# EPFL-IMOS/simple-SFOD

Hardware: AMD Instinct MI355X
Metric: teacher+student train images/s on 1024x2048 synthetic (higher is better)
Workload: dtype bf16x3

## Files before the change

include/sfod_hip.h:

```cpp
#ifndef SFOD_HIP_H
#define SFOD_HIP_H
#include <stdint.h>
#ifdef __cplusplus
extern "C" {
#endif

#define SFOD_F32 0
#define SFOD_BF16 1
#define SFOD_BF16X3 2
#define SFOD_F16X3 3

int sfod_version(void);
const char* sfod_last_error(void);

int sfod_preprocess(const void* const* img_ptrs, const int32_t* sizes, int B, int Hp, int Wp,
                    int Cpad, const float* mean3, const float* std3, void* out, int dt,
                    void* stream);

int sfod_hflip_u8(const void* src, void* dst, int C, int H, int W, void* stream);

int sfod_resize_bilinear_u8(const void* src, void* dst, int C, int H, int W, int h, int w,
                            const int32_t* hbounds, const int32_t* hcoef, int ksize_h,
                            const int32_t* vbounds, const int32_t* vcoef, int ksize_v, int flip,
                            void* stream);
int sfod_resize_bilinear_u8_opt(const void* src, void* dst, int C, int H, int W, int y0, int x0, int ch, int cw,
                                int h, int w, const int32_t* hbounds, const int32_t* hcoef, int ksize_h,
                                const int32_t* vbounds, const int32_t* vcoef, int ksize_v, int flip_mode,
                                void* stream);

int sfod_mosaic_u8(const void* const* tiles, const void* const* tabs, const int32_t* geom, int n_tiles, int fill,
                   void* out, int H0, int W0, void* stream);

int sfod_conv_fwd(const void* x, const void* w, const float* bias, void* y, int B, int H, int W,
                  int Cin, int Cout, int ksize, int ldy, int act, float* stats, int dt, int out_dt,
                  void* stream);
int sfod_conv_fwd_ws(const void* x, const void* w, const uint32_t* w_absmax, const float* bias, void* y, int B, int H,
                     int W, int Cin, int Cout, int ksize, int ldy, int act, float* stats, int dt, int out_dt,
                     void* stream);
int64_t sfod_conv_fwd_scratch_bytes(int B, int H, int W, int Cin, int Cout, int ksize, int dt, int out_dt, int with_stats);
int sfod_conv_fwd_scratch(const void* x, const void* w, const uint32_t* w_absmax, const float* bias, void* y, int B, int H,
                          int W, int Cin, int Cout, int ksize, int ldy, int act, float* stats, int dt, int out_dt,
                          void* scratch, int64_t scratch_bytes, void* stream);
int sfod_conv_stats_blocks(int B, int H, int W, int Cin, int Cout, int ksize, int dt);
int sfod_set_conv_algo(int algo);
int sfod_conv_dgrad_bnred_blocks(int B, int H, int W, int Cin, int Cout, int dt);
int sfod_conv_dgrad_bnred(const void* x, const void* w, void* dz, int B, int H, int W, int Cin, int Cout, int dt,
                          const float* y, const float* mean, const float* invstd, const float* gamma,
                          const float* beta, float* red_ws, void* stream);
int sfod_conv_fwd_bnin_supported(int B, int H, int W, int Cin, int Cout, int dt);
int sfod_conv_fwd_bnin(const float* x_pre, const float* in_mean, const float* in_invstd, const float* in_gamma,
                       const float* in_beta, const void* w, const float* bias, float* y, int B, int H, int W, int Cin,
                       int Cout, int ldy, int act, float* stats, int dt, void* stream);
int sfod_set_gemm_tile(int tile);
int sfod_set_conv3x3_variant(int variant);
int sfod_last_conv_kernel(char* buf, int n);
int sfod_set_deterministic(int on);
int sfod_get_deterministic(void);
int sfod_set_conv3x3_m16(int on);
int sfod_set_wgrad3x3_pipe(int on);
int sfod_conv_fwd_algo(int B, int H, int W, int Cin, int Cout, int ksize, int dt);

int sfod_conv_first_supported(int B, int H, int W, int Cin, int Cout, int dt, int ldy);
int sfod_conv_first_fused(const void* x, const void* w, const float* bias, const float* scale,
                          const float* shift, void* y, float* stats, int B, int H, int W, int ldy,
                          int act, int dt, void* stream);
int sfod_conv_first_fused_ws(const void* x, const void* w, const uint32_t* w_absmax, const float* bias,
                             const float* scale, const float* shift, void* y, float* stats, int B, int H, int W,
                             int ldy, int act, int dt, void* stream);
int sfod_conv_first_stats_blocks(int B, int H, int W);
int sfod_set_conv_first_pipe(int on);
int sfod_set_conv_first_grid(int n);
int sfod_conv_first_bn_apply_supported(int B, int H, int W, int Cin, int Cout, int pool_flags, int dt, int y_dt);
int sfod_conv_first_bn_apply(const void* x, const void* w, const float* bias, const float* mean, const float* invstd,
                             const float* gamma, const float* beta, void* z, int B, int H, int W, int ldz, int dt,
                             void* stream);
int sfod_set_first_apply_recompute(int on);

int64_t sfod_conv_wgrad_ws_bytes(int B, int H, int W, int Cin, int Cout, int ksize, int lddy, int dt);
int sfod_conv_wgrad(const void* x, const void* dy, float* dw, int B, int H, int W, int Cin,
                    int Cout, int ksize, int lddy, int dt, void* ws, int64_t ws_bytes, void* stream);
int sfod_conv_wgrad_oihw_supported(int B, int H, int W, int Cin, int Cout, int ksize, int lddy, int dt);
int sfod_conv_wgrad_oihw(const void* x, const void* dy, float* dw_oihw, int B, int H, int W, int Cin,
                         int Cout, int ksize, int lddy, int dt, int accumulate, void* ws,
                         int64_t ws_bytes, void* stream);
int sfod_conv_first_wgrad_bn_supported(int B, int H, int W, int Cin, int Cout, int pool, int dt, int y_dt);
int sfod_conv_first_wgrad_bn(const void* x, const void* dz, const void* y, const float* mean, const float* invstd,
                             const float* gamma, const float* beta, const float* dgamma, const float* dbeta,
                             float* dw, int B, int H, int W, int Cin, int Cout, int dt, int oihw, int accumulate,
                             void* ws, int64_t ws_bytes, void* stream);
int sfod_set_first_wgrad_fused(int on);

int sfod_pack_conv_weight(const float* w_oihw, void* w_packed, int Cout, int Cin, int ksize,
                          int CinPad, int rot180, int dt, void* stream);
int sfod_pack_conv_weight_ws(const float* w_oihw, void* w_packed, uint32_t* absmax, int Cout, int Cin, int ksize,
                             int CinPad, int rot180, int dt, void* stream);
int sfod_pack_conv_weights_blocks(int Cout, int Cin, int ksize, int innerPad, int rot180);
int sfod_pack_conv_weights_multi(const int64_t* desc, int n, int total_blocks, int dt, void* stream);
int sfod_pack_conv_weights_multi_ws(const int64_t* desc, int n, int total_blocks, int dt, uint32_t* absmax ,
                                    void* stream);
int sfod_unpack_conv_wgrad(const float* dw_packed, float* dw_oihw, int Cout, int Cin, int ksize,
                           int CinPad, int accumulate, void* stream);
int sfod_pack_fc_weight(const float* w, void* out, int N, int K, int chw_c, int transpose, int dt,
                        void* stream);
int sfod_unpack_fc_wgrad(const float* dw_packed, float* dw, int N, int K, int chw_c,
                         int accumulate, void* stream);
int sfod_pack_fc_weight_ld(const float* w, void* out, int N, int K, int chw_c, int transpose, int ld,
                           int dt, void* stream);
int sfod_pack_fc_weight_ld_ws(const float* w, void* out, uint32_t* absmax, int N, int K, int chw_c, int transpose,
                              int ld, int dt, void* stream);
int sfod_unpack_fc_wgrad_ld(const float* dw_packed, float* dw, int N, int K, int chw_c, int ld,
                            int accumulate, void* stream);
int sfod_bias_grad(const void* dy, float* db, int M, int N, int ld, int accumulate, int dt,
                   void* stream);

int sfod_bn_finalize(const float* stats, int nblocks, int M, int C,
                     float* mean, float* invstd, float* running_mean, float* running_var,
                     float momentum, float eps, int update_running, int64_t* num_batches_tracked,
                     float* ws, void* stream);
int sfod_bn_finalize_pop(const float* stats, int nblocks, int M, int C,
                         float* mean, float* invstd, float* running_mean, float* running_var,
                         float momentum, float eps, int update_running, int64_t* num_batches_tracked,
                         float* ws, double* pop, int64_t pop_stride, void* stream);
int sfod_bn_pop_commit(const double* pop, int64_t pop_stride, const int64_t* table, const int64_t* table_host, int n,
                       void* stream);
int sfod_bn_pop_merge(double* dst, const double* src, int64_t columns, void* stream);
int sfod_set_bn_finalize_fused(int on);
int sfod_bn_finalize_ws_floats(int C);
int sfod_bn_relu_pool_fwd(const void* y, const float* mean, const float* invstd,
                          const float* gamma, const float* beta, void* z, int B, int H, int W,
                          int C, int pool, int dt, int out_dt, void* stream);
int sfod_bn_relu_pool_fwd2(const void* y, const float* mean, const float* invstd,
                           const float* gamma, const float* beta, void* z, void* z2, int B, int H, int W,
                           int C, int pool, int dt, int out_dt, void* stream);
int sfod_bn_add_relu_fwd(const void* y, const float* mean, const float* invstd, const float* gamma,
                         const float* beta, const void* residual, void* z, void* z_pairs, void* z_pairs2, int64_t rows,
                         int C, int dt, int pairs_dt, void* stream);
int sfod_bn_relu_pool_bwd(const void* dz, const void* y, const float* mean, const float* invstd,
                          const float* gamma, const float* beta, void* dy, float* dgamma,
                          float* dbeta, float* dgamma_acc, float* dbeta_acc, float* ws, int B, int H,
                          int W, int C, int pool, int dt, int out_dt, int reduced_blocks, void* stream);
#define SFOD_BN_BWD_SCRATCH_ROWS 32
// ... 233 lines not shown
```

simple-sfod_amd/csrc/conv3x3_patch.hip:

```cpp
#include "conv_internal.h"
#include <type_traits>
#include <stdlib.h>

typedef __attribute__((ext_vector_type(8))) __bf16 bf16x8;
typedef __attribute__((ext_vector_type(16))) float f32x16;
typedef __attribute__((ext_vector_type(4))) float f32x4_t;

#define LDS_PTR(p) ((__attribute__((address_space(3))) void*)(p))

namespace {

template <int J> using IC = std::integral_constant<int, J>;

constexpr int BSLOT = 8192;
constexpr int STG_PITCH = 144;

template <int G, int FM> struct Lay {
  static constexpr bool SMALL = (G == 1) ? (FM == 2) : (FM == 1);
  static constexpr int NPW = SMALL ? 3 : 5;
  static constexpr int PATCH_ROWS = NPW * 8 * 16;
  static constexpr int PATCH_BYTES = PATCH_ROWS * 64;
  static constexpr int D = SMALL ? 2 : 3;
  static constexpr int NBS = D + 1;
  static constexpr int BRING_OFF = 2 * PATCH_BYTES;
// ... 506 lines not shown
      }
    }
    if (lane == 0) scnt[wave] = (float)cnt;
    __syncthreads();
    if (threadIdx.x < BN) {
      const int col = threadIdx.x;
      const int cwn = (G == 1) ? (col >> 6) : 0;
      const int cl = col & 63;
      constexpr int NWM = (G == 1) ? 4 : 8;
      double n_tot = 0.0, s_tot = 0.0;
#pragma unroll
      for (int k = 0; k < NWM; ++k) {
        const int wv = (G == 1) ? (k * 2 + cwn) : k;
        n_tot += (double)scnt[wv];
        s_tot += (double)sred[(wv * 64 + cl) * 2 + 0];
      }
      const double mu = n_tot > 0.0 ? s_tot / n_tot : 0.0;
      double m2 = 0.0;
#pragma unroll
      for (int k = 0; k < NWM; ++k) {
        const int wv = (G == 1) ? (k * 2 + cwn) : k;
        const double nk = (double)scnt[wv];
        if (nk > 0.0) {
          const double d = (double)sred[(wv * 64 + cl) * 2 + 0] / nk - mu;
          m2 += (double)sred[(wv * 64 + cl) * 2 + 1] + nk * d * d;
        }
      }
      const int n = n0 + col;
      if (n < a.Cout) {
        a.stats[((int64_t)mtile * 2 + 0) * a.Cout + n] = (float)s_tot;
        a.stats[((int64_t)mtile * 2 + 1) * a.Cout + n] = (float)m2;
      }
      if (col == 0 && tn == 0) a.stats[(int64_t)a.nblk * 2 * a.Cout + mtile] = (float)n_tot;
    }
  }
}


template <int FMT>
__device__ __forceinline__ f32x4_t mfma16(bf16x8 a, bf16x8 b, f32x4_t c) {
  if constexpr (FMT == 2)
    return __builtin_amdgcn_mfma_f32_16x16x32_f16(__builtin_bit_cast(sfod_f16x8, a), __builtin_bit_cast(sfod_f16x8, b), c, 0, 0, 0);
  else
    return __builtin_amdgcn_mfma_f32_16x16x32_bf16(a, b, c, 0, 0, 0);
}

__device__ __forceinline__ float row16_sum(float v) {
  v += __builtin_bit_cast(float, __builtin_amdgcn_update_dpp(0, __builtin_bit_cast(int, v), 0xB1, 0xF, 0xF, true));
  v += __builtin_bit_cast(float, __builtin_amdgcn_update_dpp(0, __builtin_bit_cast(int, v), 0x4E, 0xF, 0xF, true));
  v += __builtin_bit_cast(float, __builtin_amdgcn_update_dpp(0, __builtin_bit_cast(int, v), 0x141, 0xF, 0xF, true));
  v += __builtin_bit_cast(float, __builtin_amdgcn_update_dpp(0, __builtin_bit_cast(int, v), 0x140, 0xF, 0xF, true));
  return v;
}

__device__ __forceinline__ void wait_vm_dyn(int n) {
  switch (n) {
    case 0: wait_vm<0>(); break;   case 1: wait_vm<1>(); break;   case 2: wait_vm<2>(); break;   case 3: wait_vm<3>(); break;
    case 4: wait_vm<4>(); break;   case 5: wait_vm<5>(); break;   case 6: wait_vm<6>(); break;   case 7: wait_vm<7>(); break;
    case 8: wait_vm<8>(); break;   case 9: wait_vm<9>(); break;   case 10: wait_vm<10>(); break; case 11: wait_vm<11>(); break;
    case 12: wait_vm<12>(); break; case 13: wait_vm<13>(); break; case 14: wait_vm<14>(); break; default: wait_vm<15>(); break;
  }
}

template <int NW, int NIP, int NWN = 2> struct M16Lay {
  static constexpr int PIX = (NW / NWN) * NIP * 16;
  static constexpr int PR = (PIX == 256) ? 384 : 640;
  static constexpr int NPW = PR / 16 / NW;
  static constexpr int PPS = (NPW + 2) / 3;
  static constexpr int PPP = 4 * NWN;
  static constexpr int WPW = 2 * PPP / NW;
  static constexpr int PATCH_BYTES = PR * 64;
  static constexpr int WR_OFF = 2 * PATCH_BYTES;
  static constexpr int WSLOT = 2 * PPP * 1024;
  static constexpr int LDS = WR_OFF + 2 * WSLOT;
  static_assert(WPW >= 1 && PPP % WPW == 0 && PPS <= 3, "a wave's weight pieces of a stage lie inside one pair");
};

#ifdef M16_STAMP
__device__ unsigned long long g_m16_stamps[8];
#endif

typedef float __attribute__((address_space(4))) cfloat_k;

template <int NW, int NIP, int FMT, bool RED, bool XF = false, int NWN = 2>
__global__ void __launch_bounds__(NW * 64, (NW * (160 * 1024 / M16Lay<NW, NIP, NWN>::LDS)) / 4 > 0 ? (NW * (160 * 1024 / M16Lay<NW, NIP, NWN>::LDS)) / 4 : 1)
k_conv3x3_m16(P3Args a) {
  using L = M16Lay<NW, NIP, NWN>;
  static_assert(!XF || NWN == 2, "the in-LDS BatchNorm transform lives in the 128-channel shape");
  static_assert(!XF || (NW == 4 && NIP == 8 && FMT == 1 && !RED), "the in-LDS BatchNorm transform lives in the 4-wave bf16-pair forward kernel");
#ifdef M16_STAMP
  const unsigned long long stamp_t0 = __builtin_amdgcn_s_memtime();
#endif
  constexpr int PR = L::PR, NPW = L::NPW, WPW = L::WPW, PATCH_BYTES = L::PATCH_BYTES, WR_OFF = L::WR_OFF, WSLOT = L::WSLOT;
  constexpr int NWM = NW / NWN;
  constexpr int PPP = L::PPP;
  constexpr int WPX = NIP * 16;
  constexpr int XB = (NIP >= 8) ? 2 : 1;
  extern __shared__ __attribute__((aligned(16))) unsigned char smem[];

  const int lane = threadIdx.x & 63;
  const int wave = __builtin_amdgcn_readfirstlane(threadIdx.x >> 6);
  const int wm = wave / NWN, wn = wave % NWN;
  const int q = lane >> 4, r16 = lane & 15;
  const int pb = q & 1, chh = q >> 1;

  int bid = blockIdx.x;
  {
    const int qq = a.ntiles / 8, r = a.ntiles % 8, xcd = bid % 8;
    bid = (xcd < r ? xcd * (qq + 1) : r * (qq + 1) + (xcd - r) * qq) + bid / 8;
  }
  int t = (int)fdiv((unsigned)bid, (unsigned)a.tiles_n, a.m_tn);
  const int tn = bid - t * a.tiles_n;
  int t2 = (int)fdiv((unsigned)t, (unsigned)a.tiles_x, a.m_tx);
  const int txi = t - t2 * a.tiles_x;
  const int b = (int)fdiv((unsigned)t2, (unsigned)a.tiles_y, a.m_ty);
  const int tyi = t2 - b * a.tiles_y;
  const int mtile = (b * a.tiles_y + tyi) * a.tiles_x + txi;
  const int x0 = txi * a.TW, y0 = tyi * a.TH, n0 = tn * (64 * NWN);
  const int PW = a.PW;
  const int npix = a.TH * a.TW;
  const bf16_t* ximg = a.x + (int64_t)b * a.H * a.W * a.Cin;
  const int Ktot = 9 * a.Cin;

  const __amdgpu_buffer_rsrc_t xres = __builtin_amdgcn_make_buffer_rsrc((void*)ximg, (short)0, a.H * a.W * a.Cin * 2, 0x00020000);
  const __amdgpu_buffer_rsrc_t wres = __builtin_amdgcn_make_buffer_rsrc((void*)a.w, (short)0, a.Cout * Ktot * 2, 0x00020000);
  auto patch_off = [&](int k) -> unsigned {
    const int row = (wave * NPW + k) * 16 + (lane >> 2);
    const int lc = (lane & 3) ^ ((row >> 2) & 3);
    const int py = (int)fdiv((unsigned)row, (unsigned)PW, a.m_pw), px = row - py * PW;
    const int iy = y0 - 1 + py, ix = x0 - 1 + px;
    const bool ok = (py < a.TH + 2) && iy >= 0 && iy < a.H && ix >= 0 && ix < a.W;
    return ok ? (unsigned)(((iy * a.W + ix) * a.Cin + lc * 8) * 2) : OOB_OFF;
  };
  unsigned boff[WPW];
#pragma unroll
  for (int k = 0; k < WPW; ++k) {
    const int n = ((wave * WPW + k) & (PPP - 1)) * 16 + (lane >> 2);
    const int lc = (lane & 3) ^ ((n >> 2) & 3);
    boff[k] = (n0 + n < a.Cout) ? (unsigned)(((n0 + n) * Ktot + lc * 8) * 2) : OOB_OFF;
  }
  const int wpair = (wave * WPW) / PPP;
  auto issue_patch = [&](int k, int slice, int buf) {
    bufload16(xres, patch_off(k), (unsigned)__builtin_amdgcn_readfirstlane(slice * 64),
              smem + buf * PATCH_BYTES + (wave * NPW + k) * 1024);
  };
  auto issue_w = [&](int sbi, int u0, int slot) {
    const int u = u0 + wpair;
    const int sl = (u >= 9) ? 1 : 0, tap = u - 9 * sl;
    const unsigned so = (unsigned)__builtin_amdgcn_readfirstlane((tap * a.Cin + (2 * sbi + sl) * 32) * 2);
#pragma unroll
    for (int k = 0; k < WPW; ++k)
      bufload16(wres, boff[k], so, smem + WR_OFF + slot * WSLOT + (wave * WPW + k) * 1024);
  };

  const int nsb = a.nbody;
  const int nst = nsb * 9;
#pragma unroll
  for (int k = 0; k < NPW; ++k) issue_patch(k, 0, 0);
  issue_w(0, 0, 0);

  unsigned xf_valid = 0;
  int xf_row[3] = {0, 0, 0};
  const int xf_g1 = __builtin_amdgcn_readfirstlane(wave >= 2 ? 1 : 0);
  if constexpr (XF) {
    const int tid = (int)threadIdx.x;
    xf_row[0] = tid;
    xf_row[1] = (wave >= 2) ? tid - 128 : tid + 256;
    xf_row[2] = tid + 128;
#pragma unroll
    for (int k = 0; k < 3; ++k) {
      const int row = xf_row[k];
      const int py = (int)fdiv((unsigned)row, (unsigned)PW, a.m_pw), px = row - py * PW;
      const int iy = y0 - 1 + py, ix = x0 - 1 + px;
      const bool ok = (py < a.TH + 2) && iy >= 0 && iy < a.H && ix >= 0 && ix < a.W;
      xf_valid |= ok ? (1u << k) : 0u;
    }
  }
  auto transform = [&](int buf, int slice) {
    if constexpr (XF) {
      const int pbuf = buf * PATCH_BYTES;
      const int c0 = __builtin_amdgcn_readfirstlane(slice * 16);
      float4 v[3][2];
      int pa[3][2];
#pragma unroll
      for (int k = 0; k < 3; ++k) {
        const int g = (k == 0) ? 0 : (k == 2 ? 1 : xf_g1);
        const int row = xf_row[k], sw = (row >> 2) & 3;
        pa[k][0] = pbuf + row * 64 + (((2 * g) ^ sw) << 4);
        pa[k][1] = pbuf + row * 64 + (((2 * g + 1) ^ sw) << 4);
        v[k][0] = *reinterpret_cast<const float4*>(smem + pa[k][0]);
        v[k][1] = *reinterpret_cast<const float4*>(smem + pa[k][1]);
      }
#pragma unroll
      for (int k = 0; k < 3; ++k) {
        const int g = (k == 0) ? 0 : (k == 2 ? 1 : xf_g1);
        const int cb = c0 + 8 * g;
        const float yv[8] = {v[k][0].x, v[k][0].y, v[k][0].z, v[k][0].w, v[k][1].x, v[k][1].y, v[k][1].z, v[k][1].w};
        const float top = ((xf_valid >> k) & 1u) ? __builtin_inff() : 0.f;
        union { unsigned u[4]; uint4 q; } hi, lo;
        const cfloat_k* k_mean = (const cfloat_k*)(uintptr_t)a.xf_mean + cb;
        const cfloat_k* k_invstd = (const cfloat_k*)(uintptr_t)a.xf_invstd + cb;
        const cfloat_k* k_gamma = (const cfloat_k*)(uintptr_t)a.xf_gamma + cb;
        const cfloat_k* k_beta = (const cfloat_k*)(uintptr_t)a.xf_beta + cb;
#pragma unroll
        for (int e = 0; e < 8; e += 2) {
          float z[2];
#pragma unroll
          for (int i = 0; i < 2; ++i) {
            const float sc = k_invstd[e + i] * k_gamma[e + i];
            const float t = fmaf(yv[e + i] - k_mean[e + i], sc, k_beta[e + i]);
            z[i] = __builtin_amdgcn_fmed3f(t, 0.f, top);
          }
          typedef float f32x2_t __attribute__((ext_vector_type(2)));
          typedef __bf16 bf16x2_t __attribute__((ext_vector_type(2)));
          const unsigned h = __builtin_bit_cast(unsigned, __builtin_convertvector(f32x2_t{z[0], z[1]}, bf16x2_t));
          const float h0 = __builtin_bit_cast(float, h << 16), h1 = __builtin_bit_cast(float, h & 0xffff0000u);
          hi.u[e >> 1] = h;
          lo.u[e >> 1] = __builtin_bit_cast(unsigned, __builtin_convertvector(f32x2_t{z[0] - h0, z[1] - h1}, bf16x2_t));
        }
        *reinterpret_cast<uint4*>(smem + pa[k][0]) = hi.q;
        *reinterpret_cast<uint4*>(smem + pa[k][1]) = lo.q;
      }
      __builtin_amdgcn_sched_barrier(0);
    }
  };
  if constexpr (XF) {
    wait_vm<WPW>();
    __builtin_amdgcn_s_barrier();
    transform(0, 0);
  }

  int rowA[NIP];
#pragma unroll
  for (int i = 0; i < NIP; ++i) {
    const int p = wm * WPX + i * 16 + r16;
    const int ty = (int)fdiv((unsigned)p, (unsigned)a.TW, a.m_tw);
    rowA[i] = (p < npix) ? (ty * PW + (p - ty * a.TW)) : 0;
#ifdef M16_V_NOCONF
    rowA[i] = p;
#endif
    asm volatile("" : "+v"(rowA[i]));
  }
  const int offW = pb * (PPP * 1024) + (wn * 64 + r16) * 64 + (((2 * chh) ^ ((r16 >> 2) & 3)) << 4);

  f32x4_t acc[4][NIP];
#pragma unroll
  for (int i = 0; i < 4; ++i)
#pragma unroll
    for (int j = 0; j < NIP; ++j)
#pragma unroll
      for (int r = 0; r < 4; ++r) acc[i][j][r] = 0.f;

  auto stage_offq = [&](int j) -> int {
    const int ua = 2 * j, ub = 2 * j + 1;
    const int sa = (ua >= 9) ? 1 : 0, ta = ua - 9 * sa, sbb = (ub >= 9) ? 1 : 0, tb = ub - 9 * sbb;
    const int kya = (ta * 11) >> 5, kyb = (tb * 11) >> 5;
    const int dta = sa * PR + kya * PW + (ta - 3 * kya), dtb = sbb * PR + kyb * PW + (tb - 3 * kyb);
#ifdef M16_V_NOCONF
    return pb ? (dtb & ~15) : (dta & ~15);
#endif
    return pb ? dtb : dta;
  };

  {
  int sb = 0, j = 0, par = 0, nprev = 0;
#ifdef M16_V_EXTRAVALU
  int extra_valu = (int)threadIdx.x;
#endif
#ifdef M16_STAMP
  unsigned long long stamp_sum[4] = {0, 0, 0, 0};
#endif
#pragma unroll 1
  for (int g = 0; g < nst; ++g) {
    const bool last = (sb == nsb - 1);
#ifdef M16_STAMP
    const unsigned long long st_a = __builtin_amdgcn_s_memtime();
#endif
#ifndef M16_KO_BAR
    if (nprev == 0) wait_vm<0>();
    else if (nprev == 1) wait_vm<1>();
    else if (nprev == 2) wait_vm<2>();
    else wait_vm<3>();
#ifdef M16_STAMP
    const unsigned long long st_a2 = __builtin_amdgcn_s_memtime();
#endif
    __builtin_amdgcn_s_barrier();
#endif
    asm volatile("" ::: "memory");
#ifdef M16_STAMP
    const unsigned long long st_b = __builtin_amdgcn_s_memtime();
#endif
    if constexpr (XF) {
      if (j == 3) transform(1, 2 * sb + 1);
      else if (j == 8 && sb + 1 < nsb) transform(0, 2 * sb + 2);
      __builtin_amdgcn_sched_barrier(0);
    }

    const unsigned char* wsl = smem + WR_OFF + par * WSLOT;
    bf16x8 wh[4], wl[4];
#pragma unroll
    for (int ic = 0; ic < 4; ++ic) {
      wh[ic] = *reinterpret_cast<const bf16x8*>(wsl + ic * 1024 + offW);
      wl[ic] = *reinterpret_cast<const bf16x8*>(wsl + ic * 1024 + (offW ^ 16));
    }
    const int offq = stage_offq(j);
    bf16x8 xh[XB], xl[XB];
    auto read_x = [&](int ip, int slot) {
      const int row = rowA[ip] + offq;
      const int ad = row * 64 + (((2 * chh) ^ ((row >> 2) & 3)) << 4);
      xh[slot] = *reinterpret_cast<const bf16x8*>(smem + ad);
      xl[slot] = *reinterpret_cast<const bf16x8*>(smem + (ad ^ 16));
    };
    read_x(0, 0);
#if !defined(M16_KO_WDMA) && !defined(M16_V_LATEW)
    if (j < 8) issue_w(sb, 2 * j + 2, par ^ 1);
    else if (!last) issue_w(sb + 1, 0, par ^ 1);
#endif
    constexpr int PPS = XF ? (NPW + 1) / 2 : L::PPS;
    int np = 0, pslice = 0, pbuf = 0, pk = 0;
    if (j < (XF ? 2 : 3)) { pk = PPS * j; np = min(PPS, NPW - pk); pslice = 2 * sb + 1; pbuf = 1; }
    else if (j >= 5 && j < (XF ? 7 : 8) && !last) { pk = PPS * (j - 5); np = min(PPS, NPW - pk); pslice = 2 * sb + 2; pbuf = 0; }
    __builtin_amdgcn_sched_barrier(0);
#ifdef M16_STAMP
    asm volatile("s_waitcnt lgkmcnt(0)" ::: "memory");
    const unsigned long long st_c = __builtin_amdgcn_s_memtime();
    asm volatile("s_waitcnt lgkmcnt(0)" ::: "memory");
    __builtin_amdgcn_sched_barrier(0);
#endif
    __builtin_amdgcn_s_setprio(1);
#pragma unroll
    for (int ip = 0; ip < NIP; ++ip) {
      if constexpr (XB == 2) { if (ip + 1 < NIP) read_x(ip + 1, (ip + 1) & 1); }
      else { if (ip > 0) read_x(ip, 0); }
      const bf16x8 ch = xh[ip % XB], cl = xl[ip % XB];
#ifdef M16_KO_MFMA
#pragma unroll
      for (int ic = 0; ic < 4; ++ic) asm volatile("" ::"v"(wh[ic]), "v"(wl[ic]));
      asm volatile("" ::"v"(ch), "v"(cl));
      acc[0][ip][0] += 1.0f;
#else
#pragma unroll
      for (int ic = 0; ic < 4; ++ic) acc[ic][ip] = mfma16<FMT>(wh[ic], cl, acc[ic][ip]);
#pragma unroll
      for (int ic = 0; ic < 4; ++ic) acc[ic][ip] = mfma16<FMT>(wl[ic], ch, acc[ic][ip]);
#pragma unroll
      for (int ic = 0; ic < 4; ++ic) acc[ic][ip] = mfma16<FMT>(wh[ic], ch, acc[ic][ip]);
#endif
#ifndef M16_KO_PDMA
      if (ip < PPS) { if (ip < np) issue_patch(pk + ip, pslice, pbuf); }
#endif
#ifdef M16_V_EXTRAVALU
#pragma unroll
      for (int e = 0; e < (M16_V_EXTRAVALU + NIP - 1) / NIP; ++e) asm volatile("v_add_u32 %0, %0, %0" : "+v"(extra_valu));
#endif
#if defined(M16_V_LATEW) && !defined(M16_KO_WDMA)
      if (ip == 2) {
        if (j < 8) issue_w(sb, 2 * j + 2, par ^ 1);
        else if (!last) issue_w(sb + 1, 0, par ^ 1);
      }
#endif
      __builtin_amdgcn_sched_barrier(0);
    }
    __builtin_amdgcn_s_setprio(0);
#ifdef M16_STAMP
    {
      const unsigned long long st_d = __builtin_amdgcn_s_memtime();
      asm volatile("s_waitcnt lgkmcnt(0)" ::: "memory");
      stamp_sum[0] += st_a2 - st_a;
      stamp_sum[1] += st_b - st_a2;
      stamp_sum[2] += st_c - st_b;
      stamp_sum[3] += st_d - st_c;
    }
#endif
    nprev = np;
    par ^= 1;
    if (++j == 9) { j = 0; ++sb; }
  }
#ifdef M16_STAMP
  if (threadIdx.x == 0) {
    atomicAdd(&g_m16_stamps[0], stamp_sum[0]); atomicAdd(&g_m16_stamps[1], stamp_sum[1]);
    atomicAdd(&g_m16_stamps[2], stamp_sum[2]); atomicAdd(&g_m16_stamps[3], stamp_sum[3]);
    atomicAdd(&g_m16_stamps[4], (unsigned long long)nst);
    atomicAdd(&g_m16_stamps[5], __builtin_amdgcn_s_memtime() - stamp_t0);
    atomicAdd(&g_m16_stamps[6], 1ull);
  }
#endif
  }

#ifdef M16_KO_EPI
  {
    float tt = 0.f;
#pragma unroll
    for (int i = 0; i < 4; ++i)
#pragma unroll
      for (int jj = 0; jj < NIP; ++jj)
#pragma unroll
        for (int r = 0; r < 4; ++r) tt += acc[i][jj][r];
    if (tt == 1.2345e-30f) reinterpret_cast<float*>(a.y)[0] = tt;
    return;
  }
#endif
  if constexpr (FMT == 2) {
    if (a.wamax != nullptr) {
      const float inv = winv_from_absmax(*a.wamax);
#pragma unroll
      for (int i = 0; i < 4; ++i)
#pragma unroll
        for (int j = 0; j < NIP; ++j)
#pragma unroll
          for (int r = 0; r < 4; ++r) acc[i][j][r] *= inv;
    }
  }
  const ActP actp = act_params(a.act);
  const int64_t ybase = (int64_t)b * a.H * a.W;
  int pix[NIP];
#pragma unroll
  for (int ip = 0; ip < NIP; ++ip) {
    const int p = wm * WPX + ip * 16 + r16;
    int v = -1;
    if (p < npix) {
      const int ty = (int)fdiv((unsigned)p, (unsigned)a.TW, a.m_tw), tx = p - ty * a.TW;
      if (y0 + ty < a.H && x0 + tx < a.W) v = (y0 + ty) * a.W + (x0 + tx);
    }
    pix[ip] = v;
  }
  const int cb = n0 + wn * 64 + q * 4;
  float* yo = reinterpret_cast<float*>(a.y);
  const bool fast = (a.ldy % 4) == 0 && (n0 + wn * 64 + 64 <= a.Cout);
  float bv[4][4];
#pragma unroll
  for (int ic = 0; ic < 4; ++ic)
#pragma unroll
    for (int r = 0; r < 4; ++r) {
      const int c = cb + ic * 16 + r;
      bv[ic][r] = (a.bias != nullptr && c < a.Cout) ? a.bias[c] : 0.f;
    }
  int64_t rowoff[NIP];
#pragma unroll
  for (int ip = 0; ip < NIP; ++ip) rowoff[ip] = (ybase + max(pix[ip], 0)) * a.ldy;
#pragma unroll
  for (int ic = 0; ic < 4; ++ic)
#pragma unroll
    for (int ip = 0; ip < NIP; ++ip)
#pragma unroll
      for (int r = 0; r < 4; ++r) acc[ic][ip][r] += bv[ic][r];
  if (fast) {
#pragma unroll
    for (int ic = 0; ic < 4; ++ic)
#pragma unroll
      for (int ip = 0; ip < NIP; ++ip) {
        float4 o;
        o.x = act_f(acc[ic][ip][0], actp); o.y = act_f(acc[ic][ip][1], actp);
        o.z = act_f(acc[ic][ip][2], actp); o.w = act_f(acc[ic][ip][3], actp);
        if (pix[ip] >= 0) *reinterpret_cast<float4*>(yo + rowoff[ip] + (cb + ic * 16)) = o;
      }
  } else {
#pragma unroll
    for (int ic = 0; ic < 4; ++ic)
#pragma unroll
      for (int ip = 0; ip < NIP; ++ip)
#pragma unroll
        for (int r = 0; r < 4; ++r) {
          const int c = cb + ic * 16 + r;
          if (pix[ip] >= 0 && c < a.Cout) yo[rowoff[ip] + c] = act_f(acc[ic][ip][r], actp);
        }
  }

  if constexpr (!RED) { if (a.stats == nullptr) return; }
  __syncthreads();
  float* sred = reinterpret_cast<float*>(smem);
  float* scnt = sred + NW * 64 * 2;

  if constexpr (RED) {
    const float* __restrict__ yb = a.red_y + ybase * a.ldy;
#pragma unroll
    for (int ic = 0; ic < 4; ++ic) {
      const int c = cb + ic * 16;
      float mu[4], is[4], sc[4], sh[4], sbv[4], sgv[4];
#pragma unroll
      for (int r = 0; r < 4; ++r) {
        const int nc = min(c + r, a.Cout - 1);
        mu[r] = a.red_mean[nc]; is[r] = a.red_invstd[nc]; sc[r] = is[r] * a.red_gamma[nc]; sh[r] = a.red_beta[nc];
        sbv[r] = 0.f; sgv[r] = 0.f;
      }
// ... 94 lines not shown
        a.stats[((int64_t)mtile * 2 + 1) * a.Cout + n] = (float)m2;
      }
      if (col == 0 && tn == 0) a.stats[(int64_t)a.nblk * 2 * a.Cout + mtile] = (float)n_tot;
    }
  }
}

}

static SfodKnob g_p3_variant{"SFOD_P3_VARIANT", 0, [](int v) { return (v >= 1 && v <= 9) ? v : 0; }};
extern "C" int sfod_set_conv3x3_variant(int variant) { g_p3_variant.set(variant); return 0; }

static SfodKnob g_p3_m16{"SFOD_P3_M16", 1, [](int on) { return (on >= 0 && on <= 2) ? on : 1; }};
extern "C" int sfod_set_conv3x3_m16(int on) { g_p3_m16.set(on); return 0; }
static int p3_m16_n64_enabled() {
  static const int on = sfod_env_int("SFOD_P3_M16_N64", 0);
  return on;
}

static bool p3_best_tile(int H, int W, int BM, int cap, int& TH, int& TW, int& tiles_y, int& tiles_x) {
  double best = -1.0;
  for (int tw = 4; tw <= 128 && tw <= W + 3; ++tw) {
    int th = BM / tw;
    while (th > 1 && (th + 2) * (tw + 2) > cap) --th;
    if (th > H) th = H;
    if (th < 1 || (th + 2) * (tw + 2) > cap) continue;
    const int ty = (H + th - 1) / th, tx = (W + tw - 1) / tw;
    th = (H + ty - 1) / ty;
    const double eff = (double)H * W / ((double)ty * tx * (double)BM);
    const double score = eff + 1e-6 * tw + ((tw % 32 == 0) ? 0.02 : 0.0);
    if (score > best) { best = score; TH = th; TW = tw; tiles_y = ty; tiles_x = tx; }
  }
  return best >= 0.0;
}

P3Plan sfod_p3_plan(int B, int H, int W, int Cin, int Cout, int pairs) {
  P3Plan p;
  p.ok = 0;
  p.m16 = 0;
  if (H < 1 || W < 1 || B < 1) return p;
  int variant = g_p3_variant.get();
  p.m16 = (variant == 5) ? 1 : ((variant == 7 || variant == 8) ? 3 : (variant == 9 ? 4 : (variant == 6 ? 2 : (variant == 0 ? g_p3_m16.get() : 0))));
  if (variant == 5 || variant == 6) variant = 2;
  if (variant == 7 || variant == 9) variant = 3;
  if (variant == 8) variant = 4;
  if (variant < 1 || variant > 4) {
    const int64_t mt = ((int64_t)B * H * W + 255) / 256;
    const int64_t wg128 = mt * ((Cout + 127) / 128);
    variant = (Cout > 64 && wg128 >= 512) ? 2 : 3;
    if (variant == 2 && Cin >= 512 && Cout >= 512) {
      int th, tw, ty, tx;
      if (p3_best_tile(H, W, 512, PATCH_ROWS_BIG, th, tw, ty, tx)) {
        const int64_t wgs = (int64_t)B * ty * tx * ((Cout + 127) / 128);
        const int64_t rounds = (wgs + 255) / 256;
        const double px_eff = (double)H * W / ((double)ty * tx * 512.0);
        if (wgs >= 512 && (double)wgs / (double)(rounds * 256) >= 0.97 && px_eff >= 0.97) variant = 1;
      }
    }
  }
  if ((variant == 3 || variant == 4) && Cin % 64 != 0) variant = (variant == 3) ? 2 : 1;
  p.G = (variant <= 2) ? 1 : 2;
  p.FM = (variant == 1) ? 4 : (variant == 3 ? 1 : 2);
  if (Cin % (32 * p.G) != 0) return p;
  if ((int64_t)H * W * Cin >= (int64_t)1 << 30 || (int64_t)Cout * 9 * Cin >= (int64_t)1 << 30) return p;
  const int BM = (p.G == 1 ? 4 : 8) * p.FM * 32;
  const int cap = (BM == 256) ? PATCH_ROWS_SMALL : PATCH_ROWS_BIG;
  if (!p3_best_tile(H, W, BM, cap, p.TH, p.TW, p.tiles_y, p.tiles_x)) return p;
  p.tiles_n = (Cout + (128 / p.G) - 1) / (128 / p.G);
  p.nblk = B * p.tiles_y * p.tiles_x;
  p.ok = 1;
  return p;
}

#ifdef M16_STAMP
extern "C" int sfod_debug_m16_stamps(unsigned long long* out8, int reset) {
  SFOD_REQUIRE_EXTENTS("debug_m16_stamps", reset);
  hipDeviceSynchronize();
  hipMemcpyFromSymbol(out8, HIP_SYMBOL(g_m16_stamps), 64);
  if (reset) { unsigned long long z[8] = {0, 0, 0, 0, 0, 0, 0, 0}; hipMemcpyToSymbol(HIP_SYMBOL(g_m16_stamps), z, 64); }
  return 0;
}
#endif

template <int NW, int NIP, int FMT, bool RED, bool XF = false, int NWN = 2>
static int p3_launch_m16(P3Args a, hipStream_t s) {
  auto kern = k_conv3x3_m16<NW, NIP, FMT, RED, XF, NWN>;
  constexpr int LDS = M16Lay<NW, NIP, NWN>::LDS;
  static const hipError_t attr_rc =
      hipFuncSetAttribute(reinterpret_cast<const void*>(kern), hipFuncAttributeMaxDynamicSharedMemorySize, LDS);
  if (attr_rc != hipSuccess) { sfod_set_error("hipFuncSetAttribute(m16): %s", hipGetErrorString(attr_rc)); return -(int)attr_rc; }
  a.nbody = a.Cin / 64;
  static const std::string kname =
      sfod_kernel_name("k_conv3x3_m16<%d,%d,%d,%d,%d,%d>", NW, NIP, FMT, (int)RED, (int)XF, NWN);
  sfod_note_conv_kernel(kname.c_str());
  hipLaunchKernelGGL(kern, dim3(a.ntiles), dim3(NW * 64), LDS, s, a);
  return sfod_check_launch("conv3x3_m16");
}

template <int G, int FM, typename OutT, int SPLIT = 0, bool RED = false>
static int p3_launch_one(const P3Args& a, hipStream_t s) {
  auto kern = k_conv3x3_patch<G, FM, OutT, SPLIT, RED>;
  constexpr int LDS = Lay<G, FM>::TOTAL;
  static const hipError_t attr_rc =
      hipFuncSetAttribute(reinterpret_cast<const void*>(kern), hipFuncAttributeMaxDynamicSharedMemorySize, LDS);
  if (attr_rc != hipSuccess) { sfod_set_error("hipFuncSetAttribute(p3): %s", hipGetErrorString(attr_rc)); return -(int)attr_rc; }
  static const std::string kname =
      sfod_kernel_name("k_conv3x3_patch<%d,%d,%s,%d,%d>", G, FM, sfod_type_name<OutT>(), SPLIT, (int)RED);
  sfod_note_conv_kernel(kname.c_str());
  hipLaunchKernelGGL(kern, dim3(a.ntiles), dim3(512), LDS, s, a);
  return sfod_check_launch("conv3x3_patch");
}

bool sfod_p3_bnin_ok(const P3Plan& p, int Cin_phys, int split) {
  return p.ok && p.m16 != 0 && p.G == 1 && p.FM == 2 && Cin_phys % 64 == 0 && split == 1;
}

int sfod_p3_launch(const P3Plan& p, const void* x, const void* w, const float* bias, void* y, float* stats,
                   int B, int H, int W, int Cin, int Cout, int ldy, int act, int out_f32, hipStream_t s, int split,
                   const P3BnRed* red, const unsigned* wamax, const P3BnIn* bnin) {
  P3Args a;
  a.wamax = wamax;
  a.xf_mean = a.xf_invstd = a.xf_gamma = a.xf_beta = nullptr;
  if (bnin != nullptr) {
    if (!sfod_p3_bnin_ok(p, Cin, split) || red != nullptr || !out_f32) {
      sfod_set_error("conv3x3_patch: the BatchNorm-input form needs bf16x3 operands, the 256 x 128 shape, Cin % 32 == 0");
      return SFOD_EBADARG;
    }
    a.xf_mean = bnin->mean; a.xf_invstd = bnin->invstd; a.xf_gamma = bnin->gamma; a.xf_beta = bnin->beta;
  }
  a.red_y = nullptr; a.red_mean = a.red_invstd = a.red_gamma = a.red_beta = nullptr; a.red_ws = nullptr;
  if (red != nullptr) {
    if (!out_f32 || ldy != Cout || Cout % 4 != 0) { sfod_set_error("conv3x3_patch: BatchNorm-backward epilogue needs a dense fp32 output"); return SFOD_EBADARG; }
    a.red_y = red->y; a.red_mean = red->mean; a.red_invstd = red->invstd; a.red_gamma = red->gamma; a.red_beta = red->beta;
    a.red_ws = red->ws;
  }
  a.x = (const bf16_t*)x; a.w = (const bf16_t*)w; a.bias = bias; a.y = y; a.stats = stats;
  a.B = B; a.H = H; a.W = W; a.Cin = Cin; a.Cout = Cout; a.ldy = ldy; a.act = act;
  a.TH = p.TH; a.TW = p.TW; a.PW = p.TW + 2;
  a.tiles_x = p.tiles_x; a.tiles_y = p.tiles_y; a.tiles_n = p.tiles_n;
  auto magic = [](int d) { return (unsigned)((((unsigned long long)1) << 32) / (unsigned)d + 1ull); };
  a.m_pw = magic(a.PW); a.m_tw = magic(a.TW); a.m_tn = magic(a.tiles_n); a.m_tx = magic(a.tiles_x);
  a.m_ty = magic(a.tiles_y);
  a.nbody = Cin / (32 * p.G);
  a.ntiles = B * p.tiles_y * p.tiles_x * p.tiles_n;
  a.nblk = p.nblk;
  if (split) {
    if (!out_f32) { sfod_set_error("conv3x3_patch: operand pairs write fp32"); return SFOD_EBADARG; }
    if (bnin != nullptr) return p3_launch_m16<4, 8, 1, false, true>(a, s);
    if (p.m16 && p.G == 1 && p.FM == 2 && Cin % 64 == 0 && (red == nullptr || split == 1)) {
      if (p.m16 == 2) {
        if (red != nullptr) return p3_launch_m16<4, 8, 1, true>(a, s);
        return split == 2 ? p3_launch_m16<4, 8, 2, false>(a, s) : p3_launch_m16<4, 8, 1, false>(a, s);
      }
      if (red != nullptr) return p3_launch_m16<8, 4, 1, true>(a, s);
      return split == 2 ? p3_launch_m16<8, 4, 2, false>(a, s) : p3_launch_m16<8, 4, 1, false>(a, s);
    }
    if (p.m16 && p.G == 2 && Cin % 64 == 0 && (red == nullptr || split == 1) && (p.m16 >= 3 || p3_m16_n64_enabled())) {
      if (p.FM == 1 && (p.m16 == 4 || p3_m16_n64_enabled() == 2)) {
        if (red != nullptr) return p3_launch_m16<8, 2, 1, true, false, 1>(a, s);
        return split == 2 ? p3_launch_m16<8, 2, 2, false, false, 1>(a, s) : p3_launch_m16<8, 2, 1, false, false, 1>(a, s);
      }
      if (p.FM == 1) {
        if (red != nullptr) return p3_launch_m16<4, 4, 1, true, false, 1>(a, s);
        return split == 2 ? p3_launch_m16<4, 4, 2, false, false, 1>(a, s) : p3_launch_m16<4, 4, 1, false, false, 1>(a, s);
      }
      if (red != nullptr) return p3_launch_m16<8, 4, 1, true, false, 1>(a, s);
      return split == 2 ? p3_launch_m16<8, 4, 2, false, false, 1>(a, s) : p3_launch_m16<8, 4, 1, false, false, 1>(a, s);
    }
    if (red != nullptr) {
// ... 23 lines not shown
```

simple-sfod_amd/native.py:

```python
import collections
import ctypes
import math
import os
import re
import warnings

import torch

warnings.filterwarnings("ignore", message="ComplexHalf support is experimental")

_HERE = os.path.dirname(os.path.abspath(__file__))
HEADER = os.path.join(os.path.dirname(_HERE), "include", "sfod_hip.h")
SO_PATH = os.environ.get("SFOD_HIP_LIB", os.path.join(_HERE, "lib", "libsfod_hip.so"))

F32, BF16, BF16X3, F16X3 = 0, 1, 2, 3

SPLIT_DTYPE = torch.complex32
SPLITH_DTYPE = torch.uint32
PAIR_DTYPES = (SPLIT_DTYPE, SPLITH_DTYPE)

COMPUTE_MODES = {"fp32": F32, "bf16": BF16, "bf16x3": BF16X3, "f16x3": F16X3}


def mode_dt(name):
# ... 179 lines not shown
        return True


class KernelTimer:

    def __init__(self, watch=("sfod_conv_fwd", "sfod_conv_wgrad", "sfod_conv_wgrad_oihw")):
        self.watch = _Everything() if watch is None else set(watch)
        self.records = []

    def summary(self):
        torch.cuda.synchronize()
        out = {}
        for name, flops, a, b in self.records:
            d = out.setdefault(name, {"launches": 0, "ms": 0.0, "flops": 0.0})
            d["launches"] += 1
            d["ms"] += a.elapsed_time(b)
            d["flops"] += flops
        return out


_timer = None


def set_timer(timer):
    global _timer
    _timer = timer


def call(name, *args, timer_name=None, flops=0.0, tag=""):
    lib = load()
    conv = [(_p(a) if isinstance(a, torch.Tensor) else a) for a in args]
    if _timer is not None and (timer_name or name) in _timer.watch:
        a, b = torch.cuda.Event(enable_timing=True), torch.cuda.Event(enable_timing=True)
        a.record()
        rc = getattr(lib, name)(*conv, _stream())
        b.record()
        _timer.records.append(((timer_name or name) + tag, flops, a, b))
    else:
        rc = getattr(lib, name)(*conv, _stream())
    _chk(rc, name)


def query(name, *args):
    return getattr(load(), name)(*args)


def set_conv_algo(algo):
    load().sfod_set_conv_algo(int(algo))


def set_wgrad3x3_pipe(on):
    load().sfod_set_wgrad3x3_pipe(int(on))


def set_gemm_tile(tile):
    load().sfod_set_gemm_tile(int(tile))


def set_conv3x3_variant(variant):
    load().sfod_set_conv3x3_variant(int(variant))


def last_conv_kernel():
    buf = ctypes.create_string_buffer(256)
    n = load().sfod_last_conv_kernel(buf, len(buf))
    if n < 0:
        _chk(n, "sfod_last_conv_kernel")
    return buf.value.decode()


def set_deterministic(on):
    lib = load()
    prev = bool(lib.sfod_get_deterministic())
    lib.sfod_set_deterministic(int(bool(on)))
    return prev


def set_bn_finalize_fused(on):
    load().sfod_set_bn_finalize_fused(int(bool(on)))


def set_conv3x3_m16(on):
    load().sfod_set_conv3x3_m16(int(on))


_const_cache = {}


def dev_const(values, dtype, device):
    key = (values, dtype, str(device))
    t = _const_cache.get(key)
    if t is None:
        if len(_const_cache) > 4096:
            _const_cache.clear()
        t = torch.tensor(values, dtype=dtype).to(device)
        _const_cache[key] = t
    return t


_PIN_SLOTS, _PIN_WIDTH = 32, 64
_pin_ring = {}


def _pinned_upload_i64(values, dev):
    n = len(values)
    if n > _PIN_WIDTH:
        return torch.tensor(values, dtype=torch.int64).to(dev)
    st = _pin_ring.get(dev)
    if st is None:
        st = {"buf": torch.empty(_PIN_SLOTS, _PIN_WIDTH, dtype=torch.int64).pin_memory(), "ev": [None] * _PIN_SLOTS,
              "next": 0}
        _pin_ring[dev] = st
    i = st["next"]
    st["next"] = (i + 1) % _PIN_SLOTS
    if st["ev"][i] is not None:
        st["ev"][i].synchronize()
    slot = st["buf"][i, :n]
    slot.copy_(torch.tensor(values, dtype=torch.int64))
    out = slot.to(dev, non_blocking=True)
    ev = torch.cuda.Event()
    ev.record()
    st["ev"][i] = ev
    return out


def preprocess(images_u8, Hp, Wp, cpad, mean, std, dt):
    dev = images_u8[0].device
    B = len(images_u8)
    imgs = [im.contiguous() for im in images_u8]
    ptrs = _pinned_upload_i64([im.data_ptr() for im in imgs], dev)
    sizes = dev_const(tuple((int(im.shape[1]), int(im.shape[2])) for im in imgs), torch.int32, dev)
    out = torch.empty(B, Hp, Wp, cpad, dtype=torch_dtype(dt), device=dev)
    m = (ctypes.c_float * 3)(*mean)
    s = (ctypes.c_float * 3)(*std)
    lib = load()
    rc = lib.sfod_preprocess(ptrs.data_ptr(), sizes.data_ptr(), B, Hp, Wp, cpad,
                             ctypes.cast(m, ctypes.c_void_p), ctypes.cast(s, ctypes.c_void_p),
                             out.data_ptr(), dt, _stream())
    _chk(rc, "sfod_preprocess")
    out._keepalive = (imgs, ptrs)
    return out, sizes


def pil_bilinear_coeffs(in_size, out_size):
    import math
    import numpy as np
    scale = float(in_size) / float(out_size)
    filterscale = scale if scale >= 1.0 else 1.0
    support = 1.0 * filterscale
    ksize = int(math.ceil(support)) * 2 + 1
    bounds = np.zeros((out_size, 2), dtype=np.int32)
    kk = np.zeros((out_size, ksize), dtype=np.int32)
    ss = 1.0 / filterscale
    for xx in range(out_size):
        center = (xx + 0.5) * scale
        xmin = int(center - support + 0.5)
        if xmin < 0:
            xmin = 0
        xmax = int(center + support + 0.5)
        if xmax > in_size:
            xmax = in_size
        xmax -= xmin
        k = [0.0] * ksize
        ww = 0.0
        for x in range(xmax):
            a = abs((x + xmin - center + 0.5) * ss)
# ... 1319 lines not shown
```

Before: 163.2.

## Add lean variant of m16 3x3 conv kernel with precomputed offsets

Adds a LEAN template path to the m16 3x3 conv kernel. It premultiplies row offsets, keeps incremental tap and weight offset counters instead of recomputing them, precomputes patch DMA offsets, and wraps the epilogue in a compact lambda. The aim is to cut VALU address arithmetic and register pressure in the MFMA main loop. A default-on knob selects it, and for the NWN != 2 shapes it is always used. This duplicates a large amount of kernel code and adds a second compiled variant per shape.

```diff
diff --git a/include/sfod_hip.h b/include/sfod_hip.h
--- a/include/sfod_hip.h
+++ b/include/sfod_hip.h
@@ -57,6 +57,8 @@
 int sfod_set_deterministic(int on);
 int sfod_get_deterministic(void);
 int sfod_set_conv3x3_m16(int on);
+int sfod_set_conv3x3_m16_lean(int on);
+int sfod_get_conv3x3_m16_lean(void);
 int sfod_set_wgrad3x3_pipe(int on);
 int sfod_conv_fwd_algo(int B, int H, int W, int Cin, int Cout, int ksize, int dt);
 
diff --git a/simple-sfod_amd/csrc/conv3x3_patch.hip b/simple-sfod_amd/csrc/conv3x3_patch.hip
--- a/simple-sfod_amd/csrc/conv3x3_patch.hip
+++ b/simple-sfod_amd/csrc/conv3x3_patch.hip
@@ -612,7 +612,7 @@
 
 typedef float __attribute__((address_space(4))) cfloat_k;
 
-template <int NW, int NIP, int FMT, bool RED, bool XF = false, int NWN = 2>
+template <int NW, int NIP, int FMT, bool RED, bool XF = false, int NWN = 2, bool LEAN = false>
 __global__ void __launch_bounds__(NW * 64, (NW * (160 * 1024 / M16Lay<NW, NIP, NWN>::LDS)) / 4 > 0 ? (NW * (160 * 1024 / M16Lay<NW, NIP, NWN>::LDS)) / 4 : 1)
 k_conv3x3_m16(P3Args a) {
   using L = M16Lay<NW, NIP, NWN>;
@@ -766,6 +766,7 @@
     const int p = wm * WPX + i * 16 + r16;
     const int ty = (int)fdiv((unsigned)p, (unsigned)a.TW, a.m_tw);
     rowA[i] = (p < npix) ? (ty * PW + (p - ty * a.TW)) : 0;
+    if constexpr (LEAN) rowA[i] = rowA[i] * 64 + chh * 32;
 #ifdef M16_V_NOCONF
     rowA[i] = p;
 #endif
@@ -792,7 +793,121 @@
     return pb ? dtb : dta;
   };
 
-  {
+  if constexpr (LEAN) {
+  constexpr int PPS = XF ? (NPW + 1) / 2 : L::PPS;
+  constexpr int NPS = XF ? 2 : 3;
+  unsigned poff[NPW];
+#pragma unroll
+  for (int k = 0; k < NPW; ++k) { poff[k] = patch_off(k); asm volatile("" : "+v"(poff[k])); }
+  const unsigned pbm = pb ? ~0u : 0u;
+  const int PW64 = PW * 64;
+  const int wstep = 4 * a.Cin, wwrap = 64 - 18 * a.Cin;
+  int od = 0, okx = 0, ot = 0, osl = 0;
+  auto next_pair = [&]() {
+    ++ot; ++okx; od += 64;
+    if (okx == 3) { okx = 0; od += PW64 - 192; }
+    if (ot == 9) { ot = 0; osl ^= 1; od = osl ? PR * 64 : 0; }
+  };
+  int wt = wpair + 2, wso = (wpair + 2) * a.Cin * 2;
+  int sb = 0, j = 0, par = 0, nprev = 0;
+#ifdef M16_V_EXTRAVALU
+  int extra_valu = (int)threadIdx.x;
+#endif
+#pragma unroll 1
+  for (int g = 0; g < nst; ++g) {
+    const bool last = (sb == nsb - 1);
+#ifndef M16_KO_BAR
+    if (nprev == 0) wait_vm<0>();
+    else if (PPS == 1 || nprev == 1) wait_vm<1>();
+    else if (PPS == 2 || nprev == 2) wait_vm<2>();
+    else wait_vm<3>();
+    __builtin_amdgcn_s_barrier();
+#endif
+    asm volatile("" ::: "memory");
+    if constexpr (XF) {
+      if (j == 3) transform(1, 2 * sb + 1);
+      else if (j == 8 && sb + 1 < nsb) transform(0, 2 * sb + 2);
+      __builtin_amdgcn_sched_barrier(0);
+    }
+
+    const unsigned char* wsl = smem + WR_OFF + par * WSLOT;
+    bf16x8 wh[4], wl[4];
+#pragma unroll
+    for (int ic = 0; ic < 4; ++ic) {
+      wh[ic] = *reinterpret_cast<const bf16x8*>(wsl + ic * 1024 + offW);
+      wl[ic] = *reinterpret_cast<const bf16x8*>(wsl + ic * 1024 + (offW ^ 16));
+    }
+    const int oa = od;
+    next_pair();
+    const int ob = od;
+    next_pair();
+    const int offq = oa + (int)(pbm & (unsigned)(ob - oa));
+    bf16x8 xh[XB], xl[XB];
+    auto read_x = [&](int ip, int slot) {
+      const int sr = rowA[ip] + offq;
+      const int ad = sr ^ ((sr >> 4) & 0x30);
+      xh[slot] = *reinterpret_cast<const bf16x8*>(smem + ad);
+      xl[slot] = *reinterpret_cast<const bf16x8*>(smem + (ad ^ 16));
+    };
+    read_x(0, 0);
+#ifndef M16_KO_WDMA
+    if (g + 1 < nst) {
+      const unsigned so = (unsigned)__builtin_amdgcn_readfirstlane(wso);
+#pragma unroll
+      for (int k = 0; k < WPW; ++k)
+        bufload16(wres, boff[k], so, smem + WR_OFF + (par ^ 1) * WSLOT + (wave * WPW + k) * 1024);
+    }
+#endif
+    wt += 2; wso += wstep;
+    if (wt >= 9) { wt -= 9; wso += wwrap; }
+    const bool h2 = j >= 5;
+    const int jj = h2 ? j - 5 : j;
+    const int pk = PPS * jj;
+    const int np = (jj < NPS && !(h2 && last)) ? min(PPS, NPW - pk) : 0;
+    const unsigned psoff = (unsigned)__builtin_amdgcn_readfirstlane(sb * 128 + (h2 ? 128 : 64));
+    unsigned char* pdst = smem + (h2 ? 0 : PATCH_BYTES) + (wave * NPW + pk) * 1024;
+    __builtin_amdgcn_sched_barrier(0);
+    __builtin_amdgcn_s_setprio(1);
+#pragma unroll
+    for (int ip = 0; ip < NIP; ++ip) {
+      if constexpr (XB == 2) { if (ip + 1 < NIP) read_x(ip + 1, (ip + 1) & 1); }
+      else { if (ip > 0) read_x(ip, 0); }
+      const bf16x8 ch = xh[ip % XB], cl = xl[ip % XB];
+#ifdef M16_KO_MFMA
+#pragma unroll
+      for (int ic = 0; ic < 4; ++ic) asm volatile("" ::"v"(wh[ic]), "v"(wl[ic]));
+      asm volatile("" ::"v"(ch), "v"(cl));
+      acc[0][ip][0] += 1.0f;
+#else
+#pragma unroll
+      for (int ic = 0; ic < 4; ++ic) acc[ic][ip] = mfma16<FMT>(wh[ic], cl, acc[ic][ip]);
+#pragma unroll
+      for (int ic = 0; ic < 4; ++ic) acc[ic][ip] = mfma16<FMT>(wl[ic], ch, acc[ic][ip]);
+#pragma unroll
+      for (int ic = 0; ic < 4; ++ic) acc[ic][ip] = mfma16<FMT>(wh[ic], ch, acc[ic][ip]);
+#endif
+#ifndef M16_KO_PDMA
+      if (ip < PPS) {
+        if (ip < np) {
+          unsigned vo = poff[min(ip, NPW - 1)];
+          vo = (jj == 1) ? poff[min(PPS + ip, NPW - 1)] : vo;
+          if constexpr (NPS == 3) vo = (jj == 2) ? poff[min(2 * PPS + ip, NPW - 1)] : vo;
+          bufload16(xres, vo, psoff, pdst + ip * 1024);
+        }
+      }
+#endif
+#ifdef M16_V_EXTRAVALU
+#pragma unroll
+      for (int e = 0; e < (M16_V_EXTRAVALU + NIP - 1) / NIP; ++e) asm volatile("v_add_u32 %0, %0, %0" : "+v"(extra_valu));
+#endif
+      __builtin_amdgcn_sched_barrier(0);
+    }
+    __builtin_amdgcn_s_setprio(0);
+    nprev = np;
+    par ^= 1;
+    if (++j == 9) { j = 0; ++sb; }
+  }
+  } else {
   int sb = 0, j = 0, par = 0, nprev = 0;
 #ifdef M16_V_EXTRAVALU
   int extra_valu = (int)threadIdx.x;
@@ -930,6 +1045,212 @@
     return;
   }
 #endif
+  if constexpr (LEAN) {
+    const bool allv = (wm * WPX + WPX <= npix) && (y0 + a.TH <= a.H) && (x0 + a.TW <= a.W);
+    auto epilogue = [&]() {
+#pragma clang fp contract(off)
+      if constexpr (FMT == 2) {
+        if (a.wamax != nullptr) {
+          const float inv = winv_from_absmax(*a.wamax);
+#pragma unroll
+          for (int i = 0; i < 4; ++i)
+#pragma unroll
+            for (int j = 0; j < NIP; ++j)
+#pragma unroll
+              for (int r = 0; r < 4; ++r) acc[i][j][r] *= inv;
+        }
+      }
+      const ActP actp = act_params(a.act);
+      const int64_t ybase = (int64_t)b * a.H * a.W;
+      int pix[NIP];
+#pragma unroll
+      for (int ip = 0; ip < NIP; ++ip) {
+        const int p = wm * WPX + ip * 16 + r16;
+        int v = -1;
+        if (p < npix) {
+          const int ty = (int)fdiv((unsigned)p, (unsigned)a.TW, a.m_tw), tx = p - ty * a.TW;
+          if (y0 + ty < a.H && x0 + tx < a.W) v = (y0 + ty) * a.W + (x0 + tx);
+        }
+        pix[ip] = v;
+      }
+      const int cb = n0 + wn * 64 + q * 4;
+      float* yo = reinterpret_cast<float*>(a.y);
+      const bool fast = (a.ldy % 4) == 0 && (n0 + wn * 64 + 64 <= a.Cout);
+      float bv[4][4];
+#pragma unroll
+      for (int ic = 0; ic < 4; ++ic)
+#pragma unroll
+        for (int r = 0; r < 4; ++r) {
+          const int c = cb + ic * 16 + r;
+          bv[ic][r] = (a.bias != nullptr && c < a.Cout) ? a.bias[c] : 0.f;
+        }
+      int64_t rowoff[NIP];
+#pragma unroll
+      for (int ip = 0; ip < NIP; ++ip) rowoff[ip] = (ybase + max(pix[ip], 0)) * a.ldy;
+#pragma unroll
+      for (int ic = 0; ic < 4; ++ic)
+#pragma unroll
+        for (int ip = 0; ip < NIP; ++ip)
+#pragma unroll
+          for (int r = 0; r < 4; ++r) acc[ic][ip][r] += bv[ic][r];
+      if (fast) {
+#pragma unroll
+        for (int ic = 0; ic < 4; ++ic)
+#pragma unroll
+          for (int ip = 0; ip < NIP; ++ip) {
+            float4 o;
+            o.x = act_f(acc[ic][ip][0], actp); o.y = act_f(acc[ic][ip][1], actp);
+            o.z = act_f(acc[ic][ip][2], actp); o.w = act_f(acc[ic][ip][3], actp);
+            if (pix[ip] >= 0) *reinterpret_cast<float4*>(yo + rowoff[ip] + (cb + ic * 16)) = o;
+          }
+      } else {
+        int cbs = cb;
+        asm volatile("" : "+v"(cbs));
+#pragma unroll
+        for (int ic = 0; ic < 4; ++ic)
+#pragma unroll
+          for (int ip = 0; ip < NIP; ++ip)
+#pragma unroll
+            for (int r = 0; r < 4; ++r) {
+              const int c = cbs + ic * 16 + r;
+              if (pix[ip] >= 0 && c < a.Cout) yo[rowoff[ip] + c] = act_f(acc[ic][ip][r], actp);
+            }
+      }
+
+      if constexpr (!RED) { if (a.stats == nullptr) return; }
+      __syncthreads();
+      float* sred = reinterpret_cast<float*>(smem);
+      float* scnt = sred + NW * 64 * 2;
+
+      if constexpr (RED) {
+        const float* __restrict__ yb = a.red_y + ybase * a.ldy;
+        int cbr = cb;
+        asm volatile("" : "+v"(cbr));
+#pragma unroll
+        for (int ic = 0; ic < 4; ++ic) {
+          const int c = cbr + ic * 16;
+          float mu[4], is[4], sc[4], sh[4], sbv[4], sgv[4];
+#pragma unroll
+          for (int r = 0; r < 4; ++r) {
+            const int nc = min(c + r, a.Cout - 1);
+            mu[r] = a.red_mean[nc]; is[r] = a.red_invstd[nc]; sc[r] = is[r] * a.red_gamma[nc]; sh[r] = a.red_beta[nc];
+            sbv[r] = 0.f; sgv[r] = 0.f;
+          }
+          const int cc = min(c, a.Cout - 4);
+#pragma unroll
+          for (int ip = 0; ip < NIP; ++ip) {
+            const float4 yv4 = *reinterpret_cast<const float4*>(yb + (unsigned)(max(pix[ip], 0) * a.ldy + cc));
+            const float* yv = &yv4.x;
+            const bool ok = pix[ip] >= 0 && c < a.Cout;
+#pragma unroll
+            for (int r = 0; r < 4; ++r) {
+              const float d = yv[r] - mu[r];
+              const float g = (ok && fmaf(d, sc[r], sh[r]) > 0.f) ? acc[ic][ip][r] : 0.f;
+              sbv[r] += g;
+              sgv[r] = fmaf(g, d * is[r], sgv[r]);
+            }
+          }
+#pragma unroll
+          for (int r = 0; r < 4; ++r) {
+            const float s1 = row16_sum(sbv[r]), s2 = row16_sum(sgv[r]);
+            if (r16 == 0) {
+              sred[(wave * 64 + ic * 16 + q * 4 + r) * 2 + 0] = s1;
+              sred[(wave * 64 + ic * 16 + q * 4 + r) * 2 + 1] = s2;
+            }
+          }
+        }
+        __syncthreads();
+        if (threadIdx.x < 64 * NWN) {
+          const int col = threadIdx.x, cwn = col >> 6, cl = col & 63;
+          float s1 = 0.f, s2 = 0.f;
+#pragma unroll
+          for (int k = 0; k < NWM; ++k) {
+            s1 += sred[((k * NWN + cwn) * 64 + cl) * 2 + 0];
+            s2 += sred[((k * NWN + cwn) * 64 + cl) * 2 + 1];
+          }
+          const int n = n0 + col;
+          if (n < a.Cout) {
+            a.red_ws[(int64_t)mtile * 2 * a.Cout + n] = s1;
+            a.red_ws[(int64_t)mtile * 2 * a.Cout + a.Cout + n] = s2;
+          }
+        }
+        if (a.stats == nullptr) return;
+        __syncthreads();
+      }
+
+      auto wave_sums = [&](auto all_valid) {
+#pragma clang fp contract(off)
+        constexpr bool AV = decltype(all_valid)::value;
+        int cnt = WPX;
+        float inv = 1.f / (float)WPX;
+        if constexpr (!AV) {
+          cnt = 0;
+#pragma unroll
+          for (int ip = 0; ip < NIP; ++ip) cnt += (pix[ip] >= 0) ? 1 : 0;
+          cnt = (int)row16_sum((float)cnt);
+          inv = 1.f / (float)(cnt > 0 ? cnt : 1);
+        }
+#pragma unroll
+        for (int ic = 0; ic < 4; ++ic)
+#pragma unroll
+          for (int r = 0; r < 4; ++r) {
+            float s = 0.f;
+#pragma unroll
+            for (int ip = 0; ip < NIP; ++ip) s += (AV || pix[ip] >= 0) ? acc[ic][ip][r] : 0.f;
+            s = row16_sum(s);
+            float m2 = 0.f;
+#pragma unroll
+            for (int ip = 0; ip < NIP; ++ip) {
+              const float d = fmaf(-inv, s, acc[ic][ip][r]);
+              m2 += (AV || pix[ip] >= 0) ? d * d : 0.f;
+            }
+            m2 = row16_sum(m2);
+            if (r16 == 0) {
+              sred[(wave * 64 + ic * 16 + q * 4 + r) * 2 + 0] = s;
+              sred[(wave * 64 + ic * 16 + q * 4 + r) * 2 + 1] = m2;
+            }
+          }
+        if (lane == 0) scnt[wave] = (float)cnt;
+      };
+      if (allv) wave_sums(std::true_type{});
+      else wave_sums(std::false_type{});
+      __syncthreads();
+      if (threadIdx.x < 64 * NWN) {
+        const int col = threadIdx.x, cwn = col >> 6, cl = col & 63;
+        constexpr double TOT = (double)(NWM * WPX);
+        double n_tot = 0.0, s_tot = 0.0;
+#pragma unroll
+        for (int k = 0; k < NWM; ++k) {
+          const int wv = k * NWN + cwn;
+          n_tot += (double)scnt[wv];
+          s_tot += (double)sred[(wv * 64 + cl) * 2 + 0];
+        }
+        double mu = 0.0;
+        if (n_tot == TOT) mu = s_tot * (1.0 / TOT);
+        else if (n_tot == 0.5 * TOT) mu = s_tot * (2.0 / TOT);
+        else if (n_tot > 0.0) mu = s_tot / n_tot;
+        double m2 = 0.0;
+#pragma unroll
+        for (int k = 0; k < NWM; ++k) {
+          const int wv = k * NWN + cwn;
+          const double nk = (double)scnt[wv];
+          if (nk > 0.0) {
+            const double sk = (double)sred[(wv * 64 + cl) * 2 + 0];
+            const double d = (nk == (double)WPX ? sk * (1.0 / (double)WPX) : sk / nk) - mu;
+            m2 += fma(nk * d, d, (double)sred[(wv * 64 + cl) * 2 + 1]);
+          }
+        }
+        const int n = n0 + col;
+        if (n < a.Cout) {
+          a.stats[((int64_t)mtile * 2 + 0) * a.Cout + n] = (float)s_tot;
+          a.stats[((int64_t)mtile * 2 + 1) * a.Cout + n] = (float)m2;
+        }
+        if (col == 0 && tn == 0) a.stats[(int64_t)a.nblk * 2 * a.Cout + mtile] = (float)n_tot;
+      }
+    };
+    epilogue();
+    return;
+  }
   if constexpr (FMT == 2) {
     if (a.wamax != nullptr) {
       const float inv = winv_from_absmax(*a.wamax);
@@ -1190,9 +1511,24 @@
 }
 #endif
 
+static SfodKnob g_p3_m16_lean{"SFOD_M16_LEAN", 1, [](int on) { return on == 0 ? 0 : 1; }};
+extern "C" int sfod_set_conv3x3_m16_lean(int on) { g_p3_m16_lean.set(on); return 0; }
+extern "C" int sfod_get_conv3x3_m16_lean(void) { return g_p3_m16_lean.get(); }
+
+template <int NW, int NIP, int FMT, bool RED, bool XF, int NWN, bool LEAN>
+static int p3_launch_m16_body(P3Args a, hipStream_t s);
+
 template <int NW, int NIP, int FMT, bool RED, bool XF = false, int NWN = 2>
 static int p3_launch_m16(P3Args a, hipStream_t s) {
-  auto kern = k_conv3x3_m16<NW, NIP, FMT, RED, XF, NWN>;
+  if constexpr (NWN == 2) {
+    if (g_p3_m16_lean.get() == 0) return p3_launch_m16_body<NW, NIP, FMT, RED, XF, NWN, false>(a, s);
+  }
+  return p3_launch_m16_body<NW, NIP, FMT, RED, XF, NWN, true>(a, s);
+}
+
+template <int NW, int NIP, int FMT, bool RED, bool XF, int NWN, bool LEAN>
+static int p3_launch_m16_body(P3Args a, hipStream_t s) {
+  auto kern = k_conv3x3_m16<NW, NIP, FMT, RED, XF, NWN, LEAN>;
   constexpr int LDS = M16Lay<NW, NIP, NWN>::LDS;
   static const hipError_t attr_rc =
       hipFuncSetAttribute(reinterpret_cast<const void*>(kern), hipFuncAttributeMaxDynamicSharedMemorySize, LDS);
diff --git a/simple-sfod_amd/native.py b/simple-sfod_amd/native.py
--- a/simple-sfod_amd/native.py
+++ b/simple-sfod_amd/native.py
@@ -285,6 +285,13 @@
 
 def set_conv3x3_m16(on):
     load().sfod_set_conv3x3_m16(int(on))
+
+
+def set_conv3x3_m16_lean(on):
+    lib = load()
+    prev = int(lib.sfod_get_conv3x3_m16_lean())
+    lib.sfod_set_conv3x3_m16_lean(int(on))
+    return prev
 
 
 _const_cache = {}
```

Measured after the change: 164.5 (median of 6 runs). No clear change (+0.8%).
